# fr34za/multilinear

Hardware: NVIDIA B200
Metric: pcs_commit_melem_per_s (higher is better)
Workload: dtype u128

## Files before the change

### multilinear_b200/build.py

```python
import os
import shutil
import subprocess
import sys

HERE = os.path.dirname(os.path.abspath(__file__))
CSRC = os.path.join(HERE, "csrc")
OUT = os.path.join(HERE, "libmultilinear_b200.so")
SOURCES = ["core.cu", "field_ops.cu", "ntt.cu", "merkle.cu", "fri.cu", "sumcheck.cu", "mle.cu", "prover.cu", "chain.cu", "peer.cu", "shard.cu", "pcs_shard.cu"]
INSTR_OUT = os.path.join(HERE, "libmlb_instr.so")
INSTR_SOURCES = ["microbench.cu"]
HEADERS = ["field.cuh", "sha256.cuh", "reduce.cuh", "transcript.cuh", "internal.h", "handles.h", "prover_internal.h", "peer.h", os.path.join("..", "..", "include", "multilinear_b200.h"),
           os.path.join("..", "..", "include", "multilinear_b200_instr.h")]
NVCC_FLAGS = [
    "-gencode", "arch=compute_100a,code=sm_100a", "-O3", "-lineinfo", "-std=c++17", "--expt-relaxed-constexpr",
    "-Xcompiler", "-fPIC", "-diag-suppress", "177",
]


def _nvcc():
    for cand in (os.environ.get("NVCC"), shutil.which("nvcc"), "/usr/local/cuda/bin/nvcc"):
        if cand and os.path.exists(cand):
            return cand
    raise RuntimeError("nvcc not found: the CUDA extension cannot be built (there is no CPU fallback)")


def needs_build():
    if not os.path.exists(OUT) or not os.path.exists(INSTR_OUT):
        return True
    t = min(os.path.getmtime(OUT), os.path.getmtime(INSTR_OUT))
    deps = [os.path.join(CSRC, f) for f in SOURCES + INSTR_SOURCES + HEADERS] + [os.path.abspath(__file__)]
    return any(os.path.exists(d) and os.path.getmtime(d) > t for d in deps)


def build(force=False, verbose=False):
    if not force and not needs_build():
        return OUT
    nvcc = _nvcc()
    extra = os.environ.get("MLB_EXTRA_NVCC_FLAGS", "").split()
    objdir = os.path.join(HERE, "build")
    os.makedirs(objdir, exist_ok=True)
    procs = []
    for src in SOURCES + INSTR_SOURCES:
        obj = os.path.join(objdir, src.replace(".cu", ".o"))
        cmd = [nvcc] + NVCC_FLAGS + extra + ["-c", os.path.join(CSRC, src), "-o", obj]
# ... 21 lines not shown
```

### multilinear_b200/csrc/internal.h

```cpp
#pragma once
#include <atomic>
#include <cstdarg>
#include <cstdint>
#include <cstdio>
#include <cstring>
#include <map>
#include <mutex>
#include <vector>

#include <cuda_runtime.h>

#include "../../include/multilinear_b200.h"
#include "../../include/multilinear_b200_instr.h"

namespace mlb {

void set_error(const char* fmt, ...);
extern std::atomic<unsigned long long> g_kernel_launches;
#define MLB_COUNT_LAUNCH() (++::mlb::g_kernel_launches)

#define MLB_CUDA(expr)                                                                          \
    do {                                                                                        \
        cudaError_t _e = (expr);                                                                \
        if (_e != cudaSuccess) {                                                                \
// ... 59 lines not shown
    hfe r = 1;
    while (e) { if (e & 1) r = hfe_mul(r, b); b = hfe_mul(b, b); e >>= 1; }
    return r;
}
static inline hfe hfe_inv(hfe a) { return a ? hfe_pow(a, HFE_M - 2) : 0; }
static inline hfe hfe_div(hfe a, hfe b) { return hfe_mul(a, hfe_inv(b)); }
static inline hfe hfe_half(hfe a) { return hfe_mul(a, (HFE_M + 1) >> 1); }
static inline bool hfe_pow2_generator(uint64_t log_size, hfe* out) {
    if (log_size > 40) return false;
    *out = hfe_pow(3, (HFE_M - 1) >> log_size);
    return true;
}
static inline bool is_pow2(size_t n) { return n && !(n & (n - 1)); }
static inline unsigned ilog2(size_t n) { return 63u - (unsigned)__builtin_clzll((unsigned long long)n); }

struct fe;

static const int LO_BITS = 12;
struct RootTables {
    int log_n = 0;
    fe* lo = nullptr;
    fe* hi = nullptr;
    fe* lo_ninv = nullptr;
    hfe gen = 0;
    fe* pass_tw[2][4] = {{nullptr, nullptr, nullptr, nullptr}, {nullptr, nullptr, nullptr, nullptr}};
};
struct Ctx {
    int device = -1;
    cudaStream_t stream = nullptr;
    std::map<int, RootTables> roots;
    std::mutex roots_mu;
    fe* small_fwd = nullptr;
    fe* small_inv = nullptr;
    int sm_count = 148;
};
int get_ctx(Ctx** out);
cudaStream_t lib_stream(Ctx* ctx);
int lib_stream_create(cudaStream_t* out, bool non_blocking);
int lib_stream_destroy(cudaStream_t s);
int get_root_tables(Ctx* ctx, int log_n, cudaStream_t s, const RootTables** out);

int dev_alloc_async(void** p, size_t bytes, cudaStream_t s);
int dev_free_async(void* p, cudaStream_t s);

int ntt_launch(Ctx* ctx, const fe* in, fe* out, int log_n, bool inverse, bool rs_zero_padded, cudaStream_t s, bool bitrev_in = false);
static inline bool ntt_fuses_bitrev(int log_n) { return log_n > 12; }
int powers_launch(Ctx* ctx, int log_n, fe* out, cudaStream_t s);
int bit_reverse_launch(const void* in, void* out, size_t n, size_t elem_bytes, cudaStream_t s);
int fe_vec_launch(int op, const fe* a, const fe* b, size_t n, fe* out, cudaStream_t s);
int fe_pow_vec_launch(const fe* a, hfe e, size_t n, fe* out, cudaStream_t s);
int fe_from_i64_launch(const int64_t* v, size_t n, fe* out, cudaStream_t s);
int fe_from_wide_launch(const void* v, size_t n, int variant, fe* out, cudaStream_t s);
int synthetic_launch(uint64_t seed, size_t n, fe* out, cudaStream_t s);
int mobius_launch(const fe* in, fe* out, size_t len, bool subtract, cudaStream_t s);
int mle_evals_evaluate_launch(Ctx* ctx, const fe* evals, size_t len, const hfe* args, size_t n_args, hfe* out, cudaStream_t s);
int mle_coeffs_evaluate_launch(Ctx* ctx, const fe* coeffs, size_t len, const hfe* args, size_t n_args, hfe* out, cudaStream_t s);
int eq_table_launch(Ctx* ctx, const hfe* inputs, size_t n_vars, fe* delta, cudaStream_t s);
int poly_eval_launch(Ctx* ctx, const fe* coeffs, size_t n, hfe x, hfe* out, cudaStream_t s);
static inline size_t merkle_layer_offset(size_t n_leaves, size_t layer) { return 2 * n_leaves - ((2 * n_leaves) >> layer); }
int merkle_rs_launch(const fe* code, size_t n_code, uint8_t* digests, cudaStream_t s);
int merkle_bytes_launch(const uint8_t* const* data_dev_ptrs, size_t n_batches, size_t item_bytes, size_t n_items, uint8_t* digests, cudaStream_t s);
int merkle_batched_rs_launch(const fe* const* codes_dev_ptrs, size_t n_codes, size_t n_code, uint8_t* digests, cudaStream_t s);
int merkle_batched_pairs_launch(const uint8_t* const* pairs_dev_ptrs, size_t n_codes, size_t n_leaves, uint8_t* digests, cudaStream_t s);
int merkle_batched_pairs_strided_launch(const uint8_t* pairs_base, size_t n_codes, size_t n_leaves, uint8_t* digests, cudaStream_t s);
int merkle_upper_launch(uint8_t* digests, size_t n_leaves, cudaStream_t s);
int fri_fold_launch(Ctx* ctx, const fe* cur, size_t n_cur, fe* next, hfe r, const fe* r_dev, size_t k, int log_n0, cudaStream_t s);
// ... 63 lines not shown
```

### multilinear_b200/csrc/microbench.cu

```cuda
#include "field.cuh"
#include "internal.h"
#include "sha256.cuh"
#include <cstdlib>
#include <string>

namespace mlb {

template <int MODE, int V = MLB_REDUCE_V>
__global__ void __launch_bounds__(256) mb_field_kernel(fe* out, int iters, fe seed) {
    const unsigned tid = blockIdx.x * blockDim.x + threadIdx.x;
    fe a[4], w = seed;
    w.v[0] ^= tid;
#pragma unroll
    for (int i = 0; i < 4; i++) { a[i] = seed; a[i].v[1] ^= tid * 4 + i; a[i] = fe_new(a[i]); }
    w = fe_new(w);
    for (int it = 0; it < iters; it++) {
#pragma unroll
        for (int i = 0; i < 4; i += (MODE == 0 ? 1 : 2)) {
            if (MODE == 0) a[i] = fe_mul_t<V>(a[i], w);
            else {
                fe v = fe_mul_t<V>(a[i + 1], w), u = a[i];
                a[i] = fe_add(u, v);
                a[i + 1] = fe_sub(u, v);
            }
        }
    }
    fe r = fe_add(fe_add(a[0], a[1]), fe_add(a[2], a[3]));
    if (r.v[0] == 0x12345678u && r.v[3] == 0x9abcdef0u) fe_store(out + tid, r);
}
template <int MODE, int FMA_ADD, int ROT = 0, int MINB = 1>
__global__ void __launch_bounds__(128, MINB) mb_sha_kernel(uint32_t* out, int iters, uint32_t seed) {
    const unsigned tid = blockIdx.x * blockDim.x + threadIdx.x;
    uint32_t h[8], g[8];
#pragma unroll
    for (int i = 0; i < 8; i++) { h[i] = seed + tid * 8 + i; g[i] = seed ^ (tid + i); }
// ... 19 lines not shown
    uint32_t a[8], b[8];
    unsigned long long wd[8];
#pragma unroll
    for (int i = 0; i < 8; i++) { a[i] = seed + tid * 8 + i; b[i] = seed ^ (tid + 77 * i); wd[i] = a[i]; }
    uint32_t m = seed | 1u;
    double fd[8];
#pragma unroll
    for (int i = 0; i < 8; i++) fd[i] = 1.0 + 1e-9 * (double)(tid + i);
    const double fm = 1.0000001, fa = 1e-12;
    for (int it = 0; it < iters; it++) {
#pragma unroll
        for (int i = 0; i < 8; i++) {
            if (MODE == 0 || MODE == 5) asm volatile("add.u32 %0, %0, %1;" : "+r"(a[i]) : "r"(b[i]));
            if (MODE == 1 || MODE == 5 || MODE == 6 || MODE == 9) asm volatile("mad.lo.u32 %0, %0, %1, %2;" : "+r"(b[i]) : "r"(m), "r"(a[i]));
            if (MODE == 12 || MODE == 13 || MODE == 14) asm volatile("fma.rn.f64 %0, %0, %1, %2;" : "+d"(fd[i]) : "d"(fm), "d"(fa));
            if (MODE == 14) asm volatile("shf.r.wrap.b32 %0, %0, %0, 7;" : "+r"(a[i]));
            if (MODE == 2 || MODE == 7 || MODE == 13) asm volatile("{\n\t.reg .u32 lo;\n\tcvt.u32.u64 lo, %0;\n\tmad.wide.u32 %0, lo, %1, %0;\n\t}" : "+l"(wd[i]) : "r"(m));
            if (MODE == 10 || MODE == 11) asm volatile("mul.hi.u32 %0, %0, %1;" : "+r"(b[i]) : "r"(m));
            if (MODE == 11) asm volatile("shf.r.wrap.b32 %0, %0, %0, 7;" : "+r"(a[i]));
            if (MODE == 3 || MODE == 6 || MODE == 7 || MODE == 8 || MODE == 9) asm volatile("shf.r.wrap.b32 %0, %0, %0, 7;" : "+r"(a[i]));
            if (MODE == 4 || MODE == 8 || MODE == 9) asm volatile("lop3.b32 %0, %0, %1, %2, 0x96;" : "+r"(b[i]) : "r"(a[i]), "r"(m));
        }
    }
    uint32_t r = 0;
#pragma unroll
    for (int i = 0; i < 8; i++) r += a[i] + b[i] + (uint32_t)wd[i] + (uint32_t)(wd[i] >> 32) + (uint32_t)__double2uint_rz(fd[i]);
    if (r == 0x12345678u) out[tid] = r;
}

__global__ void __launch_bounds__(256) mb_copy_kernel(const uint4* __restrict__ in, uint4* __restrict__ out, size_t n) {
    size_t i = (size_t)blockIdx.x * blockDim.x + threadIdx.x;
    const size_t stride = (size_t)gridDim.x * blockDim.x;
    for (; i < n; i += stride) out[i] = __ldg(in + i);
}

}

using namespace mlb;

extern "C" int ml_microbench(const char* what, size_t n, int iters, double* ms_out, double* work_out) {
    Ctx* ctx;
    MLB_TRY(get_ctx(&ctx));
    cudaStream_t s = ctx->stream;
    cudaEvent_t e0, e1;
    MLB_CUDA(cudaEventCreate(&e0));
    MLB_CUDA(cudaEventCreate(&e1));
    void* buf = nullptr;
    const std::string w(what);
    size_t bytes = w == "copy" ? 2 * n : (n + 1024) * 16;
    MLB_CUDA(cudaMalloc(&buf, bytes));
    MLB_CUDA(cudaMemsetAsync(buf, 1, bytes, s));
    fe seed = fe{{0x9e3779b9u, 0x7f4a7c15u, 0xbf58476du, 0x14057b7eu}};
    double best = 1e30;
    for (int rep = 0; rep < 6; rep++) {
        MLB_CUDA(cudaEventRecord(e0, s));
        if (w == "modmul") mb_field_kernel<0><<<(unsigned)((n + 255) / 256), 256, 0, s>>>((fe*)buf, iters, seed);
        else if (w == "butterfly") mb_field_kernel<1><<<(unsigned)((n + 255) / 256), 256, 0, s>>>((fe*)buf, iters, seed);
        else if (w == "modmul_v1") mb_field_kernel<0, 1><<<(unsigned)((n + 255) / 256), 256, 0, s>>>((fe*)buf, iters, seed);
        else if (w == "modmul_v2") mb_field_kernel<0, 2><<<(unsigned)((n + 255) / 256), 256, 0, s>>>((fe*)buf, iters, seed);
        else if (w == "butterfly_v1") mb_field_kernel<1, 1><<<(unsigned)((n + 255) / 256), 256, 0, s>>>((fe*)buf, iters, seed);
        else if (w == "butterfly_v2") mb_field_kernel<1, 2><<<(unsigned)((n + 255) / 256), 256, 0, s>>>((fe*)buf, iters, seed);
        else if (w == "sha_leaf") mb_sha_kernel<0, MLB_SHA_ADD_MASK><<<(unsigned)((n + 127) / 128), 128, 0, s>>>((uint32_t*)buf, iters, 0x1234567u);
        else if (w == "sha_node") mb_sha_kernel<1, MLB_SHA_ADD_MASK><<<(unsigned)((n + 127) / 128), 128, 0, s>>>((uint32_t*)buf, iters, 0x1234567u);
#define MB_SHA_VARIANT(M)                                                                                                              \
        else if (w == "sha_leaf_m" #M) mb_sha_kernel<0, M><<<(unsigned)((n + 127) / 128), 128, 0, s>>>((uint32_t*)buf, iters, 0x1234567u); \
        else if (w == "sha_node_m" #M) mb_sha_kernel<1, M><<<(unsigned)((n + 127) / 128), 128, 0, s>>>((uint32_t*)buf, iters, 0x1234567u);
#define MB_SHA_ROT(M, R)                                                                                                               \
        else if (w == "sha_leaf_m" #M "_r" #R) mb_sha_kernel<0, M, R><<<(unsigned)((n + 127) / 128), 128, 0, s>>>((uint32_t*)buf, iters, 0x1234567u); \
        else if (w == "sha_node_m" #M "_r" #R) mb_sha_kernel<1, M, R><<<(unsigned)((n + 127) / 128), 128, 0, s>>>((uint32_t*)buf, iters, 0x1234567u);
        MB_SHA_ROT(2, 1) MB_SHA_ROT(2, 11) MB_SHA_ROT(2, 111) MB_SHA_ROT(2, 101) MB_SHA_ROT(2, 21) MB_SHA_ROT(2, 121) MB_SHA_ROT(2, 211)
        MB_SHA_ROT(0, 1) MB_SHA_ROT(0, 11) MB_SHA_ROT(0, 111) MB_SHA_ROT(0, 121) MB_SHA_ROT(2, 221) MB_SHA_ROT(0, 211)
        MB_SHA_VARIANT(0) MB_SHA_VARIANT(63) MB_SHA_VARIANT(3) MB_SHA_VARIANT(1) MB_SHA_VARIANT(2) MB_SHA_VARIANT(19) MB_SHA_VARIANT(11)
        MB_SHA_VARIANT(27) MB_SHA_VARIANT(59) MB_SHA_VARIANT(43)
        else if (w.rfind("pipe", 0) == 0) {
            const int mode = atoi(what + 4);
            const unsigned gb = (unsigned)((n + 255) / 256);
            switch (mode) {
                case 0: mb_pipe_kernel<0><<<gb, 256, 0, s>>>((uint32_t*)buf, iters, 0x1234567u); break;
                case 1: mb_pipe_kernel<1><<<gb, 256, 0, s>>>((uint32_t*)buf, iters, 0x1234567u); break;
                case 2: mb_pipe_kernel<2><<<gb, 256, 0, s>>>((uint32_t*)buf, iters, 0x1234567u); break;
                case 3: mb_pipe_kernel<3><<<gb, 256, 0, s>>>((uint32_t*)buf, iters, 0x1234567u); break;
                case 4: mb_pipe_kernel<4><<<gb, 256, 0, s>>>((uint32_t*)buf, iters, 0x1234567u); break;
                case 5: mb_pipe_kernel<5><<<gb, 256, 0, s>>>((uint32_t*)buf, iters, 0x1234567u); break;
                case 6: mb_pipe_kernel<6><<<gb, 256, 0, s>>>((uint32_t*)buf, iters, 0x1234567u); break;
                case 7: mb_pipe_kernel<7><<<gb, 256, 0, s>>>((uint32_t*)buf, iters, 0x1234567u); break;
                case 8: mb_pipe_kernel<8><<<gb, 256, 0, s>>>((uint32_t*)buf, iters, 0x1234567u); break;
                case 10: mb_pipe_kernel<10><<<gb, 256, 0, s>>>((uint32_t*)buf, iters, 0x1234567u); break;
                case 11: mb_pipe_kernel<11><<<gb, 256, 0, s>>>((uint32_t*)buf, iters, 0x1234567u); break;
                case 12: mb_pipe_kernel<12><<<gb, 256, 0, s>>>((uint32_t*)buf, iters, 0x1234567u); break;
                case 13: mb_pipe_kernel<13><<<gb, 256, 0, s>>>((uint32_t*)buf, iters, 0x1234567u); break;
                case 14: mb_pipe_kernel<14><<<gb, 256, 0, s>>>((uint32_t*)buf, iters, 0x1234567u); break;
                default: mb_pipe_kernel<9><<<gb, 256, 0, s>>>((uint32_t*)buf, iters, 0x1234567u); break;
            }
        }
        else if (w == "copy") mb_copy_kernel<<<148 * 16, 256, 0, s>>>((const uint4*)buf, (uint4*)((uint8_t*)buf + n), n / 16);
        else { cudaFree(buf); set_error("ml_microbench: unknown benchmark '%s'", what); return ML_ERR_ARG; }
        MLB_KERNEL_CHECK();
        MLB_CUDA(cudaEventRecord(e1, s));
        MLB_CUDA(cudaEventSynchronize(e1));
        float ms;
        MLB_CUDA(cudaEventElapsedTime(&ms, e0, e1));
        if (rep > 0 && ms < best) best = ms;
    }
    cudaFree(buf);
    cudaEventDestroy(e0);
    cudaEventDestroy(e1);
    *ms_out = best;
    if (w.rfind("modmul", 0) == 0) *work_out = (double)n * iters * 4;
    else if (w.rfind("butterfly", 0) == 0) *work_out = (double)n * iters * 2;
    else if (w == "copy") *work_out = 2.0 * (double)n;
    else if (w.rfind("pipe", 0) == 0) {
        const int mode = atoi(what + 4);
        const int per = (mode <= 4 || mode == 10 || mode == 12) ? 1 : (mode == 9 ? 3 : 2);
        *work_out = (double)n * iters * 8 * per;
    }
    else *work_out = (double)n * iters;
    return ML_OK;
}
```

### multilinear_b200/csrc/ntt.cu

```cuda
#include <cstdlib>
#include "field.cuh"
#include "internal.h"

namespace mlb {

static const int NTT_THREADS = 256;
static const int TILE_LOG = 12;

struct PassArgs {
    const fe* in;
    fe* out;
    const fe* small;
    const fe* lo;
    const fe* hi;
    const fe* wtab;
    fe scale;
    int log_n, log_r, log_t, log_a, log_b;
    int last, inverse, zero_padded, scaled_lo, has_scale;
    int bitrev_in;
    int n_passes;
    int radix_log[4];
};

template <int NS, bool LAST>
__device__ __forceinline__ void dif_round(fe* data, const fe* tw, int pitch, int log_r, int log_t, int q, int tid) {
    const int log_lr = LAST ? 0 : log_r - q - NS;
    const int items = 1 << (log_r + log_t - NS);
    for (int w = tid; w < items; w += NTT_THREADS) {
        const int t = w & ((1 << log_t) - 1);
        const int rest = w >> log_t;
        const int l = LAST ? 0 : (rest & ((1 << log_lr) - 1));
        const int blk = rest >> log_lr;
        const int m0 = (blk << (log_r - q)) + l;
        fe x[1 << NS];
#pragma unroll
        for (int j = 0; j < (1 << NS); j++) x[j] = data[(m0 + (j << log_lr)) * pitch + t];
#pragma unroll
        for (int u = 0; u < NS; u++) {
            const int span = 1 << (NS - 1 - u);
#pragma unroll
            for (int j = 0; j < (1 << NS); j++) {
                if (j & span) continue;
                fe a = x[j], b = x[j + span];
                x[j] = fe_add(a, b);
                fe d = fe_sub(a, b);
                if (LAST) {
                    if ((j & (span - 1)) != 0) d = fe_mul(d, tw[(j & (span - 1)) << (q + u)]);
                } else {
                    const int e = (((j & (span - 1)) << log_lr) + l) << (q + u);
                    d = fe_mul(d, tw[e]);
                }
                x[j + span] = d;
            }
        }
#pragma unroll
        for (int j = 0; j < (1 << NS); j++) data[(m0 + (j << log_lr)) * pitch + t] = x[j];
    }
}

__global__ void __launch_bounds__(NTT_THREADS, 3) ntt_pass_kernel(PassArgs p) {
    extern __shared__ uint4 smem_raw[];
    fe* data = reinterpret_cast<fe*>(smem_raw);
    const int R = 1 << p.log_r, T = 1 << p.log_t;
    const int pitch = (p.last && T > 1) ? T + 1 : T;
    fe* tw = data + (size_t)R * pitch;
    const int tid = threadIdx.x;
    const size_t tile = blockIdx.x;

    for (int i = tid; i < (R >> 1); i += NTT_THREADS) tw[i] = fe_load_nc(p.small + ((size_t)i << (12 - p.log_r)));
    if (tid == 0 && R == 1) tw[0] = fe_one();

    size_t a = 0, bt = 0, ap = 0, k0_base = 0;
    const int log_rb = p.log_r + p.log_b;
    if (!p.last) {
        const int log_tiles_b = p.log_b - p.log_t;
        bt = tile & (((size_t)1 << log_tiles_b) - 1);
        a = tile >> log_tiles_b;
    } else if (p.n_passes > 1) {
        const int log_k0_tiles = p.radix_log[0] - p.log_t;
        k0_base = (tile & (((size_t)1 << log_k0_tiles) - 1)) << p.log_t;
        ap = tile >> log_k0_tiles;
    }
    const int log_a_rest = p.log_a - (p.n_passes > 1 ? p.radix_log[0] : 0);

    const int tile_elems = R * T;
    if (!p.last && p.bitrev_in) {
        const int half_log = p.log_r - 1, half = R >> 1;
        for (int idx = tid; idx < half * T; idx += NTT_THREADS) {
            const int t = idx >> half_log, mp = idx & (half - 1);
            const size_t b = (bt << p.log_t) + t;
            const size_t rb = p.log_b ? (size_t)(__brevll((unsigned long long)b) >> (64 - p.log_b)) : 0;
            const int m = half_log ? (int)(__brev((unsigned)mp) >> (32 - half_log)) : 0;
            data[m * pitch + t] = fe_load_nc(p.in + (rb << half_log) + mp);
            data[(m + half) * pitch + t] = fe_zero();
        }
    } else if (!p.last) {
        const size_t base = (a << log_rb) + (bt << p.log_t);
#pragma unroll 8
        for (int idx = tid; idx < tile_elems; idx += NTT_THREADS) {
            const int t = idx & (T - 1), m = idx >> p.log_t;
            fe v;
            if (p.zero_padded && m >= (R >> 1)) v = fe_zero();
            else v = fe_load_nc(p.in + base + ((size_t)m << p.log_b) + t);
            data[m * pitch + t] = v;
        }
    } else {
#pragma unroll 8
        for (int idx = tid; idx < tile_elems; idx += NTT_THREADS) {
            const int m = idx & (R - 1), t = idx >> p.log_r;
            const size_t arow = (((k0_base + t) << log_a_rest) + ap);
            fe v;
            if (p.zero_padded && m >= (R >> 1)) v = fe_zero();
            else v = fe_load_nc(p.in + (arow << p.log_r) + m);
            data[m * pitch + t] = v;
        }
    }
    __syncthreads();

    for (int q = 0; q < p.log_r;) {
        const int rem = p.log_r - q;
        const int ns = rem % 3 ? rem % 3 : 3;
        const bool last = rem == ns;
        if (ns == 3) { if (last) dif_round<3, true>(data, tw, pitch, p.log_r, p.log_t, q, tid); else dif_round<3, false>(data, tw, pitch, p.log_r, p.log_t, q, tid); }
        else if (ns == 2) { if (last) dif_round<2, true>(data, tw, pitch, p.log_r, p.log_t, q, tid); else dif_round<2, false>(data, tw, pitch, p.log_r, p.log_t, q, tid); }
        else { if (last) dif_round<1, true>(data, tw, pitch, p.log_r, p.log_t, q, tid); else dif_round<1, false>(data, tw, pitch, p.log_r, p.log_t, q, tid); }
        q += ns;
        __syncthreads();
    }

    if (!p.last) {
        const size_t base = (a << log_rb) + (bt << p.log_t);
        const size_t nmask = ((size_t)1 << p.log_n) - 1;
#pragma unroll 4
        for (int idx = tid; idx < tile_elems; idx += NTT_THREADS) {
            const int t = idx & (T - 1), pos = idx >> p.log_t;
            const size_t k = __brev((unsigned)pos) >> (32 - p.log_r);
            const size_t b = (bt << p.log_t) + t;
            fe v = data[pos * pitch + t];
            if (p.wtab) {
                v = fe_mul(v, fe_load_nc(p.wtab + (k << p.log_b) + b));
            } else {
                size_t e = (k * b) << p.log_a;
                if (p.inverse) e = (((size_t)1 << p.log_n) - e) & nmask;
                if (e != 0 || p.scaled_lo) {
                    fe w = fe_load_nc(p.lo + (e & (((size_t)1 << LO_BITS) - 1)));
                    if (e >> LO_BITS) w = fe_mul(w, fe_load_nc(p.hi + (e >> LO_BITS)));
                    v = fe_mul(v, w);
                }
            }
            fe_store(p.out + base + (k << p.log_b) + t, v);
        }
    } else {
        size_t mid = 0;
        {
            int shift_out = 0, rem = log_a_rest;
            for (int d = 1; d < p.n_passes - 1; d++) {
                rem -= p.radix_log[d];
                const size_t kd = (ap >> rem) & (((size_t)1 << p.radix_log[d]) - 1);
                mid |= kd << shift_out;
                shift_out += p.radix_log[d];
            }
        }
        const int log_r0 = p.n_passes > 1 ? p.radix_log[0] : 0;
#pragma unroll 4
        for (int idx = tid; idx < tile_elems; idx += NTT_THREADS) {
            const int t = idx & (T - 1), pos = idx >> p.log_t;
            const size_t k = p.log_r ? (__brev((unsigned)pos) >> (32 - p.log_r)) : 0;
            fe v = data[pos * pitch + t];
            if (p.has_scale) v = fe_mul(v, p.scale);
            fe_store(p.out + (k0_base + t) + (mid << log_r0) + (k << p.log_a), v);
        }
    }
}

__global__ void root_tables_kernel(fe* lo, fe* hi, fe* lo_ninv, fe gen, fe gen_hi, fe ninv, unsigned n_lo, unsigned n_hi) {
    unsigned i = blockIdx.x * blockDim.x + threadIdx.x;
    if (i < n_lo) {
        fe w = fe_pow_u64(gen, i);
        fe_store(lo + i, w);
        fe_store(lo_ninv + i, fe_mul(w, ninv));
    }
    if (i < n_hi) fe_store(hi + i, fe_pow_u64(gen_hi, i));
}
__global__ void small_roots_kernel(fe* fwd, fe* inv, fe w, fe winv) {
    unsigned i = blockIdx.x * blockDim.x + threadIdx.x;
    if (i < 2048) {
        fe_store(fwd + i, fe_pow_u64(w, i));
        fe_store(inv + i, fe_pow_u64(winv, i));
    }
}
__global__ void pass_table_kernel(fe* out, const fe* lo, const fe* hi, int log_n, int log_a, int log_b, int inverse, size_t count) {
    size_t i = (size_t)blockIdx.x * blockDim.x + threadIdx.x;
    const size_t stride = (size_t)gridDim.x * blockDim.x;
    const size_t nmask = ((size_t)1 << log_n) - 1;
    for (; i < count; i += stride) {
        const size_t k = i >> log_b, b = i & (((size_t)1 << log_b) - 1);
        size_t e = (k * b) << log_a;
        if (inverse) e = (((size_t)1 << log_n) - e) & nmask;
        fe w = fe_load_nc(lo + (e & (((size_t)1 << LO_BITS) - 1)));
        if (e >> LO_BITS) w = fe_mul(w, fe_load_nc(hi + (e >> LO_BITS)));
        fe_store(out + i, w);
    }
}

__global__ void powers_kernel(fe* out, const fe* lo, const fe* hi, size_t n) {
// ... 55 lines not shown
    const size_t count = (size_t)1 << (log_r + log_b);
    if (count * 16 > ((size_t)1 << 30)) return ML_OK;
    static const bool no_wtab = getenv("MLB_NTT_NO_WTAB") != nullptr;
    if (no_wtab) return ML_OK;
    std::lock_guard<std::mutex> lock(ctx->roots_mu);
    RootTables& rt = ctx->roots[log_n];
    fe*& slot = rt.pass_tw[inverse ? 1 : 0][pass];
    if (!slot) {
        fe* tab;
        if (cudaMalloc((void**)&tab, count * 16) != cudaSuccess) { cudaGetLastError(); return ML_OK; }
        size_t blocks = (count + 255) / 256;
        if (blocks > (size_t)ctx->sm_count * 16) blocks = (size_t)ctx->sm_count * 16;
        const fe* lo = (inverse && pass == 0) ? rt.lo_ninv : rt.lo;
        pass_table_kernel<<<(unsigned)blocks, 256, 0, s>>>(tab, lo, rt.hi, log_n, log_a, log_b, inverse ? 1 : 0, count);
        MLB_KERNEL_CHECK();
        MLB_CUDA(cudaStreamSynchronize(s));
        slot = tab;
    }
    *out = slot;
    return ML_OK;
}

int powers_launch(Ctx* ctx, int log_n, fe* out, cudaStream_t s) {
    const RootTables* rt;
    MLB_TRY(get_root_tables(ctx, log_n, s, &rt));
    const size_t n = (size_t)1 << log_n;
    size_t blocks = (n + 255) / 256;
    if (blocks > (size_t)ctx->sm_count * 16) blocks = (size_t)ctx->sm_count * 16;
    powers_kernel<<<(unsigned)blocks, 256, 0, s>>>(out, rt->lo, rt->hi, n);
    MLB_KERNEL_CHECK();
    return ML_OK;
}

int ntt_launch(Ctx* ctx, const fe* in, fe* out, int log_n, bool inverse, bool rs_zero_padded, cudaStream_t s, bool bitrev_in) {
    if (bitrev_in && !(rs_zero_padded && !inverse && log_n > TILE_LOG)) { set_error("ntt: bit-reversed input needs a multi-pass RS encode"); return ML_ERR_ARG; }
    MLB_CUDA(cudaFuncSetAttribute(ntt_pass_kernel, cudaFuncAttributeMaxDynamicSharedMemorySize, 112 * 1024));
    const RootTables* rt;
    MLB_TRY(get_root_tables(ctx, log_n, s, &rt));
    if (log_n == 0) {
        if (in != out) MLB_CUDA(cudaMemcpyAsync(out, in, 16, cudaMemcpyDeviceToDevice, s));
        return ML_OK;
    }
    int n_passes = log_n <= TILE_LOG ? 1 : (log_n + 8) / 9;
    int radix_log[4] = {0, 0, 0, 0};
    if (n_passes > 4) { set_error("NTT size 2^%d not supported", log_n); return ML_ERR_ARG; }
    for (int p = 0; p < n_passes; p++) radix_log[p] = log_n / n_passes + (p < log_n % n_passes ? 1 : 0);

    struct TmpGuard {
        fe* p = nullptr;
        cudaStream_t s;
        explicit TmpGuard(cudaStream_t st) : s(st) {}
        ~TmpGuard() { if (p) cudaFreeAsync(p, s); }
    } tmp_guard(s);
    if (n_passes > 1) MLB_TRY(dev_alloc_async((void**)&tmp_guard.p, ((size_t)16) << log_n, s));
    fe* const tmp = tmp_guard.p;

    const double nbytes = 16.0 * (double)((size_t)1 << log_n);
    ProfScope prof(PROF_NTT_PASS, rs_zero_padded ? 1.5 * nbytes : 2.0 * nbytes, s);
    PassArgs a;
    memset(&a, 0, sizeof a);
    a.small = inverse ? ctx->small_inv : ctx->small_fwd;
    a.hi = rt->hi;
    a.log_n = log_n;
    a.inverse = inverse ? 1 : 0;
    a.n_passes = n_passes;
    for (int p = 0; p < 4; p++) a.radix_log[p] = radix_log[p];
    int log_a = 0;
    for (int p = 0; p < n_passes; p++) {
        a.last = p == n_passes - 1;
        a.in = p == 0 ? in : tmp;
        a.out = a.last ? out : tmp;
        a.log_r = radix_log[p];
        a.log_a = log_a;
        a.log_b = log_n - log_a - a.log_r;
        a.log_t = n_passes == 1 ? 0 : TILE_LOG - a.log_r;
        a.zero_padded = (rs_zero_padded && p == 0) ? 1 : 0;
        a.bitrev_in = (bitrev_in && p == 0) ? 1 : 0;
        a.scaled_lo = (inverse && p == 0 && n_passes > 1) ? 1 : 0;
        a.lo = a.scaled_lo ? rt->lo_ninv : rt->lo;
        a.wtab = nullptr;
        if (!a.last) MLB_TRY(get_pass_table(ctx, log_n, inverse, p, a.log_a, a.log_r, a.log_b, s, &a.wtab));
        a.has_scale = (inverse && n_passes == 1) ? 1 : 0;
        if (a.has_scale) a.scale = to_dev_fe(hfe_inv(hfe_new((hfe)1 << log_n)));
        const int R = 1 << a.log_r, T = 1 << a.log_t;
        const int pitch = (a.last && T > 1) ? T + 1 : T;
        const size_t smem = ((size_t)R * pitch + (R >> 1) + 1) * 16;
        const size_t tiles = ((size_t)1 << log_n) >> (a.log_r + a.log_t);
        ntt_pass_kernel<<<(unsigned)tiles, NTT_THREADS, smem, s>>>(a);
        MLB_KERNEL_CHECK();
        log_a += a.log_r;
    }
    return ML_OK;
}

__global__ void bit_reverse_kernel(const uint4* in, uint4* out, size_t n, int bits) {
    size_t i = (size_t)blockIdx.x * blockDim.x + threadIdx.x;
    const size_t stride = (size_t)gridDim.x * blockDim.x;
    for (; i < n; i += stride) {
        size_t j = (bits && (i >> bits) == 0) ? (size_t)(__brevll((unsigned long long)i) >> (64 - bits)) : i;
        out[i] = in[j];
    }
}
int bit_reverse_launch(const void* in, void* out, size_t n, size_t elem_bytes, cudaStream_t s) {
    if (elem_bytes != 16) { set_error("bit_reverse: device path handles 16-byte elements"); return ML_ERR_ARG; }
    if (n == 0) return ML_OK;
    int bits = __builtin_ctzll((unsigned long long)n);
    size_t blocks = (n + 255) / 256;
    if (blocks > 148 * 32) blocks = 148 * 32;
    ProfScope prof(PROF_BITREV, 32.0 * (double)n, s);
    bit_reverse_kernel<<<(unsigned)blocks, 256, 0, s>>>((const uint4*)in, (uint4*)out, n, bits);
    MLB_KERNEL_CHECK();
    return ML_OK;
}

}
```

Measured before the change: 1879.

## Run radix-256/512 NTT passes as 16-point DFTs on tcgen05 int8 tensor cores

New measurement: 1831, median of 6. 2.6% lower.

```diff
diff --git a/_prof.py b/_prof.py
--- /dev/null
+++ b/_prof.py
@@ -0,0 +1,20 @@
+import ctypes as C, json, os, sys, collections
+sys.path.insert(0, os.path.dirname(os.path.abspath(__file__)))
+import torch
+from torch.profiler import profile, ProfilerActivity
+from multilinear_b200 import api as ml
+from multilinear_b200 import load
+log_n = int(sys.argv[1]); L = load(); ml.set_device(0)
+n = 1 << log_n
+c = ml.synthetic_elements_dev(0xB200, n); out = ml.DeviceBuffer(32 * n)
+g = ml.pow_2_generator(log_n + 1); gb = (C.c_uint8 * 16)(*g.to_bytes(16, "little"))
+for _ in range(3): ml.check(L.ml_reed_solomon_dev(c.ptr, C.c_size_t(n), gb, out.ptr, None))
+ml.synchronize()
+with profile(activities=[ProfilerActivity.CUDA]) as prof:
+    for _ in range(10): ml.check(L.ml_reed_solomon_dev(c.ptr, C.c_size_t(n), gb, out.ptr, None))
+    ml.synchronize()
+seq = [(e.name, e.device_time) for e in prof.events() if e.device_type.name == "CUDA" and "ntt" in e.name]
+per = len(seq) // 10
+tot = collections.defaultdict(float)
+for i, (nm, t) in enumerate(seq): tot[(i % per, nm[:40])] += t / 10
+print(json.dumps({"tc": os.environ.get("MLB_NTT_TC", "1"), "log_n": log_n, "passes_us": [[k[0], k[1], round(v, 1)] for k, v in sorted(tot.items())]}))
diff --git a/multilinear_b200/build.py b/multilinear_b200/build.py
--- a/multilinear_b200/build.py
+++ b/multilinear_b200/build.py
@@ -9,7 +9,7 @@
 SOURCES = ["core.cu", "field_ops.cu", "ntt.cu", "merkle.cu", "fri.cu", "sumcheck.cu", "mle.cu", "prover.cu", "chain.cu", "peer.cu", "shard.cu", "pcs_shard.cu"]
 INSTR_OUT = os.path.join(HERE, "libmlb_instr.so")
 INSTR_SOURCES = ["microbench.cu"]
-HEADERS = ["field.cuh", "sha256.cuh", "reduce.cuh", "transcript.cuh", "internal.h", "handles.h", "prover_internal.h", "peer.h", os.path.join("..", "..", "include", "multilinear_b200.h"),
+HEADERS = ["field.cuh", "tc.cuh", "sha256.cuh", "reduce.cuh", "transcript.cuh", "internal.h", "handles.h", "prover_internal.h", "peer.h", os.path.join("..", "..", "include", "multilinear_b200.h"),
            os.path.join("..", "..", "include", "multilinear_b200_instr.h")]
 NVCC_FLAGS = [
     "-gencode", "arch=compute_100a,code=sm_100a", "-O3", "-lineinfo", "-std=c++17", "--expt-relaxed-constexpr",
diff --git a/multilinear_b200/csrc/internal.h b/multilinear_b200/csrc/internal.h
--- a/multilinear_b200/csrc/internal.h
+++ b/multilinear_b200/csrc/internal.h
@@ -115,6 +115,7 @@
     std::mutex roots_mu;
     fe* small_fwd = nullptr;
     fe* small_inv = nullptr;
+    void* dft16_b[2] = {nullptr, nullptr};
     int sm_count = 148;
 };
 int get_ctx(Ctx** out);
diff --git a/multilinear_b200/csrc/microbench.cu b/multilinear_b200/csrc/microbench.cu
--- a/multilinear_b200/csrc/microbench.cu
+++ b/multilinear_b200/csrc/microbench.cu
@@ -1,6 +1,7 @@
 #include "field.cuh"
 #include "internal.h"
 #include "sha256.cuh"
+#include "tc.cuh"
 #include <cstdlib>
 #include <string>
 
@@ -86,6 +87,46 @@
     size_t i = (size_t)blockIdx.x * blockDim.x + threadIdx.x;
     const size_t stride = (size_t)gridDim.x * blockDim.x;
     for (; i < n; i += stride) out[i] = __ldg(in + i);
+}
+
+__global__ void __launch_bounds__(128, 1) mb_utcimma_kernel(uint32_t* out, int iters, uint32_t seed) {
+    extern __shared__ uint4 mb_smem[];
+    uint8_t* a = reinterpret_cast<uint8_t*>(mb_smem);
+    uint8_t* b = a + 128 * 256;
+    __shared__ uint64_t mbar;
+    __shared__ uint32_t tslot;
+    for (int i = threadIdx.x; i < (128 + 256) * 256 / 16; i += blockDim.x) {
+        uint32_t h = (seed ^ (uint32_t)i) * 0x9E3779B1u;
+        mb_smem[i] = make_uint4(h, h * 0x85EBCA77u, h * 0xC2B2AE3Du, h ^ 0x27D4EB2Fu);
+    }
+    fence_proxy_async_smem();
+    if (threadIdx.x < 32) tc_alloc(&tslot, 512);
+    if (threadIdx.x == 0) mbar_init(&mbar, 1);
+    tc_fence_before_sync();
+    __syncthreads();
+    tc_fence_after_sync();
+    const uint32_t tmem = tslot;
+    if (threadIdx.x == 0) {
+        const uint32_t sa = smem_u32(a), sb = smem_u32(b), idesc = tc_idesc_u8(128, 256);
+        for (int it = 0; it < iters; it++) {
+#pragma unroll
+            for (int s = 0; s < 8; s++)
+                tc_mma_u8(tmem + (uint32_t)(it & 1) * 256, tc_smem_desc(sa + s * 2 * 2048, 2048, 128), tc_smem_desc(sb + s * 2 * 4096, 4096, 128),
+                          idesc, s > 0);
+        }
+        tc_commit(&mbar);
+    }
+    mbar_wait(&mbar, 0);
+    tc_fence_after_sync();
+    uint32_t r[64];
+    tc_ld64(tmem + ((uint32_t)(threadIdx.x & 96) << 16), r);
+    uint32_t x = 0;
+#pragma unroll
+    for (int i = 0; i < 64; i++) x += r[i];
+    if (x == 0x12345678u) out[threadIdx.x] = x;
+    tc_fence_before_sync();
+    __syncthreads();
+    if (threadIdx.x < 32) tc_dealloc(tmem, 512);
 }
 
 }
@@ -147,6 +188,10 @@
                 default: mb_pipe_kernel<9><<<gb, 256, 0, s>>>((uint32_t*)buf, iters, 0x1234567u); break;
             }
         }
+        else if (w == "utcimma") {
+            MLB_CUDA(cudaFuncSetAttribute(mb_utcimma_kernel, cudaFuncAttributeMaxDynamicSharedMemorySize, (128 + 256) * 256));
+            mb_utcimma_kernel<<<(unsigned)n, 128, (128 + 256) * 256, s>>>((uint32_t*)buf, iters, 0x1234567u);
+        }
         else if (w == "copy") mb_copy_kernel<<<148 * 16, 256, 0, s>>>((const uint4*)buf, (uint4*)((uint8_t*)buf + n), n / 16);
         else { cudaFree(buf); set_error("ml_microbench: unknown benchmark '%s'", what); return ML_ERR_ARG; }
         MLB_KERNEL_CHECK();
@@ -163,6 +208,7 @@
     if (w.rfind("modmul", 0) == 0) *work_out = (double)n * iters * 4;
     else if (w.rfind("butterfly", 0) == 0) *work_out = (double)n * iters * 2;
     else if (w == "copy") *work_out = 2.0 * (double)n;
+    else if (w == "utcimma") *work_out = (double)n * iters * 128.0 * 256.0 * 256.0;
     else if (w.rfind("pipe", 0) == 0) {
         const int mode = atoi(what + 4);
         const int per = (mode <= 4 || mode == 10 || mode == 12) ? 1 : (mode == 9 ? 3 : 2);
diff --git a/multilinear_b200/csrc/ntt.cu b/multilinear_b200/csrc/ntt.cu
--- a/multilinear_b200/csrc/ntt.cu
+++ b/multilinear_b200/csrc/ntt.cu
@@ -1,6 +1,9 @@
+#include <algorithm>
 #include <cstdlib>
+#include <cstring>
 #include "field.cuh"
 #include "internal.h"
+#include "tc.cuh"
 
 namespace mlb {
 
@@ -58,44 +61,40 @@
     }
 }
 
-__global__ void __launch_bounds__(NTT_THREADS, 3) ntt_pass_kernel(PassArgs p) {
-    extern __shared__ uint4 smem_raw[];
-    fe* data = reinterpret_cast<fe*>(smem_raw);
-    const int R = 1 << p.log_r, T = 1 << p.log_t;
-    const int pitch = (p.last && T > 1) ? T + 1 : T;
-    fe* tw = data + (size_t)R * pitch;
-    const int tid = threadIdx.x;
-    const size_t tile = blockIdx.x;
-
-    for (int i = tid; i < (R >> 1); i += NTT_THREADS) tw[i] = fe_load_nc(p.small + ((size_t)i << (12 - p.log_r)));
-    if (tid == 0 && R == 1) tw[0] = fe_one();
-
-    size_t a = 0, bt = 0, ap = 0, k0_base = 0;
-    const int log_rb = p.log_r + p.log_b;
+struct TileCoord {
+    size_t a, bt, ap, k0_base;
+};
+__device__ __forceinline__ TileCoord tile_coord(const PassArgs& p, size_t tile) {
+    TileCoord c{0, 0, 0, 0};
     if (!p.last) {
         const int log_tiles_b = p.log_b - p.log_t;
-        bt = tile & (((size_t)1 << log_tiles_b) - 1);
-        a = tile >> log_tiles_b;
+        c.bt = tile & (((size_t)1 << log_tiles_b) - 1);
+        c.a = tile >> log_tiles_b;
     } else if (p.n_passes > 1) {
         const int log_k0_tiles = p.radix_log[0] - p.log_t;
-        k0_base = (tile & (((size_t)1 << log_k0_tiles) - 1)) << p.log_t;
-        ap = tile >> log_k0_tiles;
-    }
-    const int log_a_rest = p.log_a - (p.n_passes > 1 ? p.radix_log[0] : 0);
-
+        c.k0_base = (tile & (((size_t)1 << log_k0_tiles) - 1)) << p.log_t;
+        c.ap = tile >> log_k0_tiles;
+    }
+    return c;
+}
+__device__ __forceinline__ int log_a_rest(const PassArgs& p) { return p.log_a - (p.n_passes > 1 ? p.radix_log[0] : 0); }
+
+__device__ __forceinline__ void load_tile(const PassArgs& p, fe* data, int pitch, const TileCoord& c, int tid) {
+    const int R = 1 << p.log_r, T = 1 << p.log_t;
     const int tile_elems = R * T;
+    const int log_rb = p.log_r + p.log_b;
     if (!p.last && p.bitrev_in) {
         const int half_log = p.log_r - 1, half = R >> 1;
         for (int idx = tid; idx < half * T; idx += NTT_THREADS) {
             const int t = idx >> half_log, mp = idx & (half - 1);
-            const size_t b = (bt << p.log_t) + t;
+            const size_t b = (c.bt << p.log_t) + t;
             const size_t rb = p.log_b ? (size_t)(__brevll((unsigned long long)b) >> (64 - p.log_b)) : 0;
             const int m = half_log ? (int)(__brev((unsigned)mp) >> (32 - half_log)) : 0;
             data[m * pitch + t] = fe_load_nc(p.in + (rb << half_log) + mp);
             data[(m + half) * pitch + t] = fe_zero();
         }
     } else if (!p.last) {
-        const size_t base = (a << log_rb) + (bt << p.log_t);
+        const size_t base = (c.a << log_rb) + (c.bt << p.log_t);
 #pragma unroll 8
         for (int idx = tid; idx < tile_elems; idx += NTT_THREADS) {
             const int t = idx & (T - 1), m = idx >> p.log_t;
@@ -105,37 +104,37 @@
             data[m * pitch + t] = v;
         }
     } else {
+        const int lar = log_a_rest(p);
 #pragma unroll 8
         for (int idx = tid; idx < tile_elems; idx += NTT_THREADS) {
             const int m = idx & (R - 1), t = idx >> p.log_r;
-            const size_t arow = (((k0_base + t) << log_a_rest) + ap);
+            const size_t arow = (((c.k0_base + t) << lar) + c.ap);
             fe v;
             if (p.zero_padded && m >= (R >> 1)) v = fe_zero();
             else v = fe_load_nc(p.in + (arow << p.log_r) + m);
             data[m * pitch + t] = v;
         }
     }
-    __syncthreads();
-
-    for (int q = 0; q < p.log_r;) {
-        const int rem = p.log_r - q;
-        const int ns = rem % 3 ? rem % 3 : 3;
-        const bool last = rem == ns;
-        if (ns == 3) { if (last) dif_round<3, true>(data, tw, pitch, p.log_r, p.log_t, q, tid); else dif_round<3, false>(data, tw, pitch, p.log_r, p.log_t, q, tid); }
-        else if (ns == 2) { if (last) dif_round<2, true>(data, tw, pitch, p.log_r, p.log_t, q, tid); else dif_round<2, false>(data, tw, pitch, p.log_r, p.log_t, q, tid); }
-        else { if (last) dif_round<1, true>(data, tw, pitch, p.log_r, p.log_t, q, tid); else dif_round<1, false>(data, tw, pitch, p.log_r, p.log_t, q, tid); }
-        q += ns;
-        __syncthreads();
-    }
-
+}
+
+template <bool TC>
+__device__ __forceinline__ size_t out_digit(const PassArgs& p, int pos, int h) {
+    if (TC) return p.log_r == 9 ? (size_t)((pos << 1) | h) : (size_t)pos;
+    return p.log_r ? (__brev((unsigned)pos) >> (32 - p.log_r)) : 0;
+}
+
+template <bool TC>
+__device__ __forceinline__ void store_tile(const PassArgs& p, const fe* data, int pitch, const TileCoord& c, int tid, int h = 0) {
+    const int T = 1 << p.log_t;
+    const int tile_elems = T << ((TC && p.log_r == 9) ? 8 : p.log_r);
     if (!p.last) {
-        const size_t base = (a << log_rb) + (bt << p.log_t);
+        const size_t base = (c.a << (p.log_r + p.log_b)) + (c.bt << p.log_t);
         const size_t nmask = ((size_t)1 << p.log_n) - 1;
 #pragma unroll 4
         for (int idx = tid; idx < tile_elems; idx += NTT_THREADS) {
             const int t = idx & (T - 1), pos = idx >> p.log_t;
-            const size_t k = __brev((unsigned)pos) >> (32 - p.log_r);
-            const size_t b = (bt << p.log_t) + t;
+            const size_t k = out_digit<TC>(p, pos, h);
+            const size_t b = (c.bt << p.log_t) + t;
             fe v = data[pos * pitch + t];
             if (p.wtab) {
                 v = fe_mul(v, fe_load_nc(p.wtab + (k << p.log_b) + b));
@@ -153,10 +152,10 @@
     } else {
         size_t mid = 0;
         {
-            int shift_out = 0, rem = log_a_rest;
+            int shift_out = 0, rem = log_a_rest(p);
             for (int d = 1; d < p.n_passes - 1; d++) {
                 rem -= p.radix_log[d];
-                const size_t kd = (ap >> rem) & (((size_t)1 << p.radix_log[d]) - 1);
+                const size_t kd = (c.ap >> rem) & (((size_t)1 << p.radix_log[d]) - 1);
                 mid |= kd << shift_out;
                 shift_out += p.radix_log[d];
             }
@@ -165,12 +164,198 @@
 #pragma unroll 4
         for (int idx = tid; idx < tile_elems; idx += NTT_THREADS) {
             const int t = idx & (T - 1), pos = idx >> p.log_t;
-            const size_t k = p.log_r ? (__brev((unsigned)pos) >> (32 - p.log_r)) : 0;
+            const size_t k = out_digit<TC>(p, pos, h);
             fe v = data[pos * pitch + t];
             if (p.has_scale) v = fe_mul(v, p.scale);
-            fe_store(p.out + (k0_base + t) + (mid << log_r0) + (k << p.log_a), v);
-        }
-    }
+            fe_store(p.out + (c.k0_base + t) + (mid << log_r0) + (k << p.log_a), v);
+        }
+    }
+}
+
+__global__ void __launch_bounds__(NTT_THREADS, 3) ntt_pass_kernel(PassArgs p) {
+    extern __shared__ uint4 smem_raw[];
+    fe* data = reinterpret_cast<fe*>(smem_raw);
+    const int R = 1 << p.log_r, T = 1 << p.log_t;
+    const int pitch = (p.last && T > 1) ? T + 1 : T;
+    fe* tw = data + (size_t)R * pitch;
+    const int tid = threadIdx.x;
+
+    for (int i = tid; i < (R >> 1); i += NTT_THREADS) tw[i] = fe_load_nc(p.small + ((size_t)i << (12 - p.log_r)));
+    if (tid == 0 && R == 1) tw[0] = fe_one();
+
+    const TileCoord c = tile_coord(p, blockIdx.x);
+    load_tile(p, data, pitch, c, tid);
+    __syncthreads();
+
+    for (int q = 0; q < p.log_r;) {
+        const int rem = p.log_r - q;
+        const int ns = rem % 3 ? rem % 3 : 3;
+        const bool last = rem == ns;
+        if (ns == 3) { if (last) dif_round<3, true>(data, tw, pitch, p.log_r, p.log_t, q, tid); else dif_round<3, false>(data, tw, pitch, p.log_r, p.log_t, q, tid); }
+        else if (ns == 2) { if (last) dif_round<2, true>(data, tw, pitch, p.log_r, p.log_t, q, tid); else dif_round<2, false>(data, tw, pitch, p.log_r, p.log_t, q, tid); }
+        else { if (last) dif_round<1, true>(data, tw, pitch, p.log_r, p.log_t, q, tid); else dif_round<1, false>(data, tw, pitch, p.log_r, p.log_t, q, tid); }
+        q += ns;
+        __syncthreads();
+    }
+
+    store_tile<false>(p, data, pitch, c, tid);
+}
+
+static const int TC_LOG_T = 3;
+
+__global__ void dft16_b_kernel(uint8_t* out, const fe* small) {
+    const int i = blockIdx.x * blockDim.x + threadIdx.x;
+    if (i >= 4096) return;
+    const int k = i >> 8, j = (i >> 4) & 15, b = i & 15;
+    const int x = (j * k) & 15;
+    fe w = fe_load_nc(small + ((x & 7) << 8));
+    if (x & 8) w = fe_neg(w);
+    fe s = fe_zero();
+    s.v[b >> 2] = 1u << (8 * (b & 3));
+    const fe v = fe_mul(w, s);
+#pragma unroll
+    for (int e = 0; e < 16; e++) {
+        const int n = 16 * k + e;
+        out[((j * 32) + (n >> 3)) * 128 + (n & 7) * 16 + b] = (uint8_t)(v.v[e >> 2] >> (8 * (e & 3)));
+    }
+}
+
+__device__ __forceinline__ fe tc_reassemble(const uint32_t (&c)[16]) {
+    uint32_t l[4], cin = 0;
+#pragma unroll
+    for (int L = 0; L < 4; L++) {
+        const uint32_t c0 = c[4 * L], c1 = c[4 * L + 1], c2 = c[4 * L + 2], c3 = c[4 * L + 3];
+        uint32_t x, h;
+        asm("add.cc.u32 %0, %2, %3; addc.u32 %1, %4, %5;\n\t"
+            "add.cc.u32 %0, %0, %6; addc.u32 %1, %1, 0;\n\t"
+            "add.cc.u32 %0, %0, %7; addc.u32 %1, %1, 0;\n\t"
+            "add.cc.u32 %0, %0, %8; addc.u32 %1, %1, 0;"
+            : "=&r"(x), "=&r"(h)
+            : "r"(c0), "r"(c1 << 8), "r"(c2 >> 16), "r"(c3 >> 8), "r"(c2 << 16), "r"(c3 << 24), "r"(cin));
+        l[L] = x;
+        cin = h;
+    }
+    const uint32_t top = cin, t1 = top * MLB_K45;
+    uint32_t y0, y1, y2, y3, k2, k1;
+    asm("sub.cc.u32 %0, %5, %9; subc.cc.u32 %1, %6, 0; subc.cc.u32 %2, %7, 0; subc.cc.u32 %3, %8, 0; subc.u32 %4, 0, 0;"
+        : "=&r"(y0), "=&r"(y1), "=&r"(y2), "=&r"(y3), "=&r"(k2) : "r"(l[0]), "r"(l[1]), "r"(l[2]), "r"(l[3]), "r"(top));
+    asm("add.cc.u32 %0, %0, %4; addc.cc.u32 %1, %1, 0; addc.cc.u32 %2, %2, 0; addc.u32 %3, 0, 0;"
+        : "+r"(y1), "+r"(y2), "+r"(y3), "=&r"(k1) : "r"(t1));
+    uint32_t z0, z1, z2, z3, g;
+    asm("add.cc.u32 %0, %5, %9; addc.cc.u32 %1, %6, %10; addc.cc.u32 %2, %7, 0; addc.cc.u32 %3, %8, 0; addc.u32 %4, %11, %12;"
+        : "=&r"(z0), "=&r"(z1), "=&r"(z2), "=&r"(z3), "=&r"(g)
+        : "r"(y0), "r"(y1), "r"(y2), "r"(y3), "r"(MLB_C0), "r"(MLB_C1), "r"(k1), "r"(k2));
+    return fe{{g ? z0 : y0, g ? z1 : y1, g ? z2 : y2, g ? z3 : y3}};
+}
+
+__device__ __forceinline__ void tc_load_half(const PassArgs& p, fe* data, int pitch, const TileCoord& c, int h, const fe* tw, int tid) {
+    const int T = 1 << TC_LOG_T;
+    if (p.bitrev_in) {
+        for (int idx = tid; idx < 256 * T; idx += NTT_THREADS) {
+            const int t = idx >> 8, mp = idx & 255;
+            const size_t b = (c.bt << p.log_t) + t;
+            const size_t rb = p.log_b ? (size_t)(__brevll((unsigned long long)b) >> (64 - p.log_b)) : 0;
+            const int m = (int)(__brev((unsigned)mp) >> 24);
+            const fe v = fe_load_nc(p.in + (rb << 8) + mp);
+            data[m * pitch + t] = h ? fe_mul(v, tw[m]) : v;
+        }
+        return;
+    }
+    const int lar = log_a_rest(p);
+    for (int idx = tid; idx < 256 * T; idx += NTT_THREADS) {
+        int t, m;
+        const fe* src;
+        if (p.last) {
+            m = idx & 255, t = idx >> 8;
+            src = p.in + ((((c.k0_base + t) << lar) + c.ap) << p.log_r) + m;
+        } else {
+            t = idx & (T - 1), m = idx >> TC_LOG_T;
+            src = p.in + (c.a << (p.log_r + p.log_b)) + (c.bt << p.log_t) + ((size_t)m << p.log_b) + t;
+        }
+        const fe u = fe_load_nc(src);
+        fe v;
+        if (p.zero_padded) {
+            v = h ? fe_mul(u, tw[m]) : u;
+        } else {
+            const fe w = fe_load_nc(src + (p.last ? (size_t)256 : ((size_t)256 << p.log_b)));
+            v = h ? fe_mul(fe_sub(u, w), tw[m]) : fe_add(u, w);
+        }
+        data[m * pitch + t] = v;
+    }
+}
+
+__global__ void __launch_bounds__(NTT_THREADS, 2) ntt_pass_tc_kernel(PassArgs p, const uint4* gb, size_t tiles) {
+    extern __shared__ uint4 smem_raw[];
+    uint4* gs = smem_raw;
+    fe* data = reinterpret_cast<fe*>(smem_raw + 4096);
+    const int R = 1 << p.log_r;
+    const int pitch = p.last ? (1 << TC_LOG_T) + 1 : (1 << TC_LOG_T);
+    fe* tw = data + 256 * pitch;
+    uint64_t* mbar = reinterpret_cast<uint64_t*>(tw + R);
+    uint32_t* tslot = reinterpret_cast<uint32_t*>(mbar + 1);
+    const int tid = threadIdx.x, warp = tid >> 5;
+
+    for (int i = tid; i < 4096; i += NTT_THREADS) gs[i] = __ldg(gb + i);
+    for (int i = tid; i < R; i += NTT_THREADS) {
+        const int hi = i >= (R >> 1);
+        const fe w = fe_load_nc(p.small + ((size_t)(i - (hi ? R >> 1 : 0)) << (12 - p.log_r)));
+        tw[i] = hi ? fe_neg(w) : w;
+    }
+    if (warp == 0) tc_alloc(tslot, 256);
+    if (tid == 0) mbar_init(mbar, 1);
+    tc_fence_before_sync();
+    __syncthreads();
+    tc_fence_after_sync();
+    const uint32_t tmem = *tslot;
+    uint32_t phase = 0;
+
+    const uint32_t sg = smem_u32(gs), sdata = smem_u32(data), row = (uint32_t)pitch * 16;
+    const uint32_t idesc = tc_idesc_u8(128, 256);
+    const int inst = ((warp & 3) << 5) | (tid & 31);
+    const int g = inst >> 3, t = inst & 7, k_lo = (warp >> 2) << 3;
+    const uint32_t tlane = tmem + ((uint32_t)((warp & 3) << 5) << 16);
+
+    const int log_halves = p.log_r - 8;
+    for (size_t item = blockIdx.x; item < (tiles << log_halves); item += gridDim.x) {
+        const TileCoord c = tile_coord(p, item >> log_halves);
+        const int h = (int)(item & (((size_t)1 << log_halves) - 1));
+        if (log_halves) tc_load_half(p, data, pitch, c, h, tw, tid);
+        else load_tile(p, data, pitch, c, tid);
+#pragma unroll 1
+        for (int level = 0; level < 2; level++) {
+            fence_proxy_async_smem();
+            tc_fence_before_sync();
+            __syncthreads();
+            if (tid == 0) {
+                tc_fence_after_sync();
+#pragma unroll
+                for (int s = 0; s < 8; s++)
+                    tc_mma_u8(tmem, tc_smem_desc(sdata + 2 * s * 16 * row, 16 * row, row), tc_smem_desc(sg + 2 * s * 4096, 4096, 128), idesc, s > 0);
+                tc_commit(mbar);
+            }
+            mbar_wait(mbar, phase);
+            phase ^= 1;
+            tc_fence_after_sync();
+#pragma unroll 1
+            for (int kq = 0; kq < 8; kq += 4) {
+                uint32_t acc[64];
+                tc_ld64(tlane + (uint32_t)(k_lo + kq) * 16, acc);
+#pragma unroll
+                for (int u = 0; u < 4; u++) {
+                    const int k = k_lo + kq + u;
+                    fe y = tc_reassemble(*reinterpret_cast<const uint32_t(*)[16]>(acc + 16 * u));
+                    if (level == 0) data[(16 * g + k) * pitch + t] = fe_mul(y, tw[((k * g) & 255) << log_halves]);
+                    else data[(g + 16 * k) * pitch + t] = y;
+                }
+            }
+        }
+        __syncthreads();
+        store_tile<true>(p, data, pitch, c, tid, h);
+        __syncthreads();
+    }
+    tc_fence_before_sync();
+    __syncthreads();
+    if (warp == 0) tc_dealloc(tmem, 256);
 }
 
 __global__ void root_tables_kernel(fe* lo, fe* hi, fe* lo_ninv, fe gen, fe gen_hi, fe ninv, unsigned n_lo, unsigned n_hi) {
@@ -292,9 +477,26 @@
     return ML_OK;
 }
 
+static int get_dft16_b(Ctx* ctx, bool inverse, cudaStream_t s, const uint4** out) {
+    std::lock_guard<std::mutex> lock(ctx->roots_mu);
+    void*& slot = ctx->dft16_b[inverse ? 1 : 0];
+    if (!slot) {
+        void* tab;
+        MLB_CUDA(cudaMalloc(&tab, 65536));
+        dft16_b_kernel<<<16, 256, 0, s>>>((uint8_t*)tab, inverse ? ctx->small_inv : ctx->small_fwd);
+        MLB_KERNEL_CHECK();
+        MLB_CUDA(cudaStreamSynchronize(s));
+        slot = tab;
+    }
+    *out = (const uint4*)slot;
+    return ML_OK;
+}
+
 int ntt_launch(Ctx* ctx, const fe* in, fe* out, int log_n, bool inverse, bool rs_zero_padded, cudaStream_t s, bool bitrev_in) {
     if (bitrev_in && !(rs_zero_padded && !inverse && log_n > TILE_LOG)) { set_error("ntt: bit-reversed input needs a multi-pass RS encode"); return ML_ERR_ARG; }
     MLB_CUDA(cudaFuncSetAttribute(ntt_pass_kernel, cudaFuncAttributeMaxDynamicSharedMemorySize, 112 * 1024));
+    MLB_CUDA(cudaFuncSetAttribute(ntt_pass_tc_kernel, cudaFuncAttributeMaxDynamicSharedMemorySize, 160 * 1024));
+    static const bool tc_off = [] { const char* e = getenv("MLB_NTT_TC"); return e && strcmp(e, "0") == 0; }();
     const RootTables* rt;
     MLB_TRY(get_root_tables(ctx, log_n, s, &rt));
     if (log_n == 0) {
@@ -333,7 +535,8 @@
         a.log_r = radix_log[p];
         a.log_a = log_a;
         a.log_b = log_n - log_a - a.log_r;
-        a.log_t = n_passes == 1 ? 0 : TILE_LOG - a.log_r;
+        const bool tc = !tc_off && n_passes > 1 && (a.log_r == 8 || a.log_r == 9);
+        a.log_t = n_passes == 1 ? 0 : tc ? TC_LOG_T : TILE_LOG - a.log_r;
         a.zero_padded = (rs_zero_padded && p == 0) ? 1 : 0;
         a.bitrev_in = (bitrev_in && p == 0) ? 1 : 0;
         a.scaled_lo = (inverse && p == 0 && n_passes > 1) ? 1 : 0;
@@ -344,9 +547,20 @@
         if (a.has_scale) a.scale = to_dev_fe(hfe_inv(hfe_new((hfe)1 << log_n)));
         const int R = 1 << a.log_r, T = 1 << a.log_t;
         const int pitch = (a.last && T > 1) ? T + 1 : T;
-        const size_t smem = ((size_t)R * pitch + (R >> 1) + 1) * 16;
         const size_t tiles = ((size_t)1 << log_n) >> (a.log_r + a.log_t);
-        ntt_pass_kernel<<<(unsigned)tiles, NTT_THREADS, smem, s>>>(a);
+        if (tc) {
+            const uint4* gb;
+            MLB_TRY(get_dft16_b(ctx, inverse, s, &gb));
+            const size_t smem = 65536 + ((size_t)256 * pitch + R) * 16 + 16;
+            int per_sm = 0;
+            MLB_CUDA(cudaOccupancyMaxActiveBlocksPerMultiprocessor(&per_sm, ntt_pass_tc_kernel, NTT_THREADS, smem));
+            const size_t items = tiles << (a.log_r - 8);
+            const size_t grid = std::min(items, (size_t)ctx->sm_count * (size_t)(per_sm > 0 ? per_sm : 1));
+            ntt_pass_tc_kernel<<<(unsigned)grid, NTT_THREADS, smem, s>>>(a, gb, tiles);
+        } else {
+            const size_t smem = ((size_t)R * pitch + (R >> 1) + 1) * 16;
+            ntt_pass_kernel<<<(unsigned)tiles, NTT_THREADS, smem, s>>>(a);
+        }
         MLB_KERNEL_CHECK();
         log_a += a.log_r;
     }
diff --git a/multilinear_b200/csrc/tc.cuh b/multilinear_b200/csrc/tc.cuh
--- /dev/null
+++ b/multilinear_b200/csrc/tc.cuh
@@ -0,0 +1,68 @@
+#pragma once
+#include <cstdint>
+#include <cuda_runtime.h>
+
+namespace mlb {
+
+__device__ __forceinline__ uint32_t smem_u32(const void* p) { return (uint32_t)__cvta_generic_to_shared(p); }
+
+__device__ __forceinline__ uint64_t tc_smem_desc(uint32_t saddr, uint32_t lbo, uint32_t sbo) {
+    return (uint64_t)((saddr >> 4) & 0x3FFFu) | ((uint64_t)((lbo >> 4) & 0x3FFFu) << 16) | ((uint64_t)((sbo >> 4) & 0x3FFFu) << 32) |
+           ((uint64_t)1 << 46);
+}
+
+__host__ __device__ constexpr uint32_t tc_idesc_u8(int m, int n) { return (2u << 4) | ((uint32_t)(n >> 3) << 17) | ((uint32_t)(m >> 4) << 24); }
+
+__device__ __forceinline__ void tc_mma_u8(uint32_t d_tmem, uint64_t a_desc, uint64_t b_desc, uint32_t idesc, bool accumulate) {
+    asm volatile(
+        "{\n\t.reg .pred p;\n\tsetp.ne.b32 p, %4, 0;\n\t"
+        "tcgen05.mma.cta_group::1.kind::i8 [%0], %1, %2, %3, p;\n\t}"
+        :: "r"(d_tmem), "l"(a_desc), "l"(b_desc), "r"(idesc), "r"((uint32_t)accumulate));
+}
+
+__device__ __forceinline__ void tc_commit(uint64_t* mbar) {
+    asm volatile("tcgen05.commit.cta_group::1.mbarrier::arrive::one.shared::cluster.b64 [%0];" :: "r"(smem_u32(mbar)) : "memory");
+}
+
+__device__ __forceinline__ void mbar_init(uint64_t* mbar, uint32_t count) {
+    asm volatile("mbarrier.init.shared::cta.b64 [%0], %1;" :: "r"(smem_u32(mbar)), "r"(count) : "memory");
+    asm volatile("fence.mbarrier_init.release.cluster;" ::: "memory");
+}
+
+__device__ __forceinline__ void mbar_wait(uint64_t* mbar, uint32_t phase) {
+    asm volatile(
+        "{\n\t.reg .pred done;\n"
+        "WAIT_%=:\n\t"
+        "mbarrier.try_wait.parity.shared::cta.b64 done, [%0], %1;\n\t"
+        "@!done bra WAIT_%=;\n\t}"
+        :: "r"(smem_u32(mbar)), "r"(phase) : "memory");
+}
+
+__device__ __forceinline__ void fence_proxy_async_smem() { asm volatile("fence.proxy.async.shared::cta;" ::: "memory"); }
+__device__ __forceinline__ void tc_fence_before_sync() { asm volatile("tcgen05.fence::before_thread_sync;" ::: "memory"); }
+__device__ __forceinline__ void tc_fence_after_sync() { asm volatile("tcgen05.fence::after_thread_sync;" ::: "memory"); }
+
+__device__ __forceinline__ void tc_alloc(uint32_t* slot, uint32_t cols) {
+    asm volatile("tcgen05.alloc.cta_group::1.sync.aligned.shared::cta.b32 [%0], %1;" :: "r"(smem_u32(slot)), "r"(cols) : "memory");
+    asm volatile("tcgen05.relinquish_alloc_permit.cta_group::1.sync.aligned;" ::: "memory");
+}
+__device__ __forceinline__ void tc_dealloc(uint32_t taddr, uint32_t cols) {
+    asm volatile("tcgen05.dealloc.cta_group::1.sync.aligned.b32 %0, %1;" :: "r"(taddr), "r"(cols) : "memory");
+}
+
+__device__ __forceinline__ void tc_ld64(uint32_t taddr, uint32_t (&r)[64]) {
+    asm volatile(
+        "tcgen05.ld.sync.aligned.32x32b.x64.b32 {%0, %1, %2, %3, %4, %5, %6, %7, %8, %9, %10, %11, %12, %13, %14, %15, %16, %17, %18, %19, %20, %21, %22, %23, %24, %25, %26, %27, %28, %29, %30, %31, %32, %33, %34, %35, %36, %37, %38, %39, %40, %41, %42, %43, %44, %45, %46, %47, %48, %49, %50, %51, %52, %53, %54, %55, %56, %57, %58, %59, %60, %61, %62, %63}, [%64];\n\t"
+        "tcgen05.wait::ld.sync.aligned;"
+        : "=r"(r[0]), "=r"(r[1]), "=r"(r[2]), "=r"(r[3]), "=r"(r[4]), "=r"(r[5]), "=r"(r[6]), "=r"(r[7]),
+          "=r"(r[8]), "=r"(r[9]), "=r"(r[10]), "=r"(r[11]), "=r"(r[12]), "=r"(r[13]), "=r"(r[14]), "=r"(r[15]),
+          "=r"(r[16]), "=r"(r[17]), "=r"(r[18]), "=r"(r[19]), "=r"(r[20]), "=r"(r[21]), "=r"(r[22]), "=r"(r[23]),
+          "=r"(r[24]), "=r"(r[25]), "=r"(r[26]), "=r"(r[27]), "=r"(r[28]), "=r"(r[29]), "=r"(r[30]), "=r"(r[31]),
+          "=r"(r[32]), "=r"(r[33]), "=r"(r[34]), "=r"(r[35]), "=r"(r[36]), "=r"(r[37]), "=r"(r[38]), "=r"(r[39]),
+          "=r"(r[40]), "=r"(r[41]), "=r"(r[42]), "=r"(r[43]), "=r"(r[44]), "=r"(r[45]), "=r"(r[46]), "=r"(r[47]),
+          "=r"(r[48]), "=r"(r[49]), "=r"(r[50]), "=r"(r[51]), "=r"(r[52]), "=r"(r[53]), "=r"(r[54]), "=r"(r[55]),
+          "=r"(r[56]), "=r"(r[57]), "=r"(r[58]), "=r"(r[59]), "=r"(r[60]), "=r"(r[61]), "=r"(r[62]), "=r"(r[63])
+        : "r"(taddr) : "memory");
+}
+
+}
```
